# GeekAlexis/FastMOT

Hardware: AMD Instinct MI355X
Metric: end-to-end tracker FPS @1080p/50 dets (higher is better)
Workload: dtype f16

## Files before the change

### fastmot_amd/csrc/net.h

```cpp
#pragma once
#include "common.h"
#include <hip/hip_fp16.h>

typedef _Float16 f16;
typedef f16 f16x8 __attribute__((ext_vector_type(8)));
typedef f16 f16x4 __attribute__((ext_vector_type(4)));
typedef float f32x16 __attribute__((ext_vector_type(16)));
typedef float f32x4 __attribute__((ext_vector_type(4)));

enum { ACT_LINEAR = 0, ACT_LEAKY = 1, ACT_MISH = 2, ACT_RELU = 3, ACT_LOGISTIC = 4, ACT_SWISH = 5, ACT_RELU6 = 6 };
enum { RES_NONE = 0, RES_AFTER_ACT = 1, RES_BEFORE_ACT = 2 };

struct ConvParams {
    const f16* in;  int in_cs, in_coff;
    const f16* w;
    const float* bias;
    f16* out;       int out_cs, out_coff;
    float* out32;
    const f16* res; int res_cs, res_coff;
    int N, H, W, Cin, Ho, Wo, Cout, KH, KW, stride, pad;
    int K, Kpad, P;
    int cout_store;
    int act, res_mode;
    int grid_p, grid_c, grid_z, weight_major;
    int pad_dx;
    int up;
    int batch_inv;
};

int launch_conv(const ConvParams& p, float* ws, size_t ws_floats, hipStream_t s);

struct NetState {
    int which = 0, max_batch = 0;
    std::vector<fm_tensor> tensors;
    std::vector<void*> bufs;
    std::vector<fm_layer> layers;
    char* weights = nullptr;
    size_t weight_bytes = 0;
    float* gates = nullptr;
    int n_gates = 0, gate_c = 0;
    hipStream_t stream = nullptr;
    char* arena = nullptr;
    float* ws = nullptr;
    size_t ws_floats = 0;
    std::vector<std::pair<long, hipGraphExec_t>> graphs;
    bool use_graphs = true;
    int emb_offset = 0;
    int batch_offset = 0;
    int first = 0;
};

NetState* fm_net_get(fm_ctx* ctx, int which);
int fm_net_run_internal(fm_ctx* ctx, int which, int batch);

__device__ __forceinline__ void unpack8(const uint4& v, float* f) {
    const f16x8 h = *reinterpret_cast<const f16x8*>(&v);
#pragma unroll
    for (int e = 0; e < 8; ++e) f[e] = (float)h[e];
}
__device__ __forceinline__ uint4 pack8(const float* f) {
    f16x8 h;
#pragma unroll
    for (int e = 0; e < 8; ++e) h[e] = (f16)f[e];
    return *reinterpret_cast<const uint4*>(&h);
// ... 107 lines not shown
```

### fastmot_amd/csrc/net.hip

```cpp
#include "pixel_source.h"
#include <algorithm>
#include <memory>

int launch_dwconv3(const f16* in, int in_cs, int in_coff, f16* out, int out_cs, int out_coff, const f16* w,
                   const float* bias, int N, int H, int W, int C, int act, hipStream_t s);
int launch_dwconv(const f16* in, int in_cs, int in_coff, f16* out, int out_cs, int out_coff, const f16* w,
                  const float* bias, int N, int H, int W, int Ho, int Wo, int C, int stride, int act, hipStream_t s);
bool sepconv_supported(int cin, int cout, int stride);
int launch_sepconv(const f16* in, int in_cs, int in_coff, f16* out, int out_cs, int out_coff, const f16* wdw,
                   const float* bdw, const f16* wpw, const float* bpw, int N, int H, int W, int Ho, int Wo, int cin,
                   int cout, int stride, int act1, int act2, long p_choice, hipStream_t s);
int launch_liteconv(int G, const f16* const* in, const int* in_cs, const int* in_coff, f16* out, int out_cs,
                    int out_coff, const f16* wpw, int kpad, const f16* wdw, const float* bias, int N, int H,
                    int W, int C, int act, float* gap_out, hipStream_t s);
void liteconv_tiling(int C, int W, int H, int* th, int* tw, int* tiles_x, int* tiles_y);
int launch_litechain(const f16* in, int in_cs, int in_coff, f16* out, int out_cs, int out_coff, const f16* wpw,
                     int kpad, const f16* wdw, const float* bias, int N, int H, int W, int C, int act,
                     float* const* gap, hipStream_t s);
int launch_gated_sum(int nstreams, const f16* const* in, const int* in_cs, const int* in_coff, int N, int HW,
                     int C, int hid, const f16* w1, const float* b1, const f16* w2, const float* b2, f16* out,
                     int out_cs, int out_coff, const float* const* part, int tiles, hipStream_t s);
constexpr int GATE_SLOT_TILES = 32;
int launch_pair11(const f16* xa, int xa_cs, int xa_coff, const f16* xc, int xc_cs, int xc_coff, f16* out, int out_cs,
                  int out_coff, const f16* w1, const float* b1, const f16* w2, const float* b2, long P, int cout, int act1,
// ... 4 lines not shown
bool ostail_supported(int in_h, int in_w, int cin, int mid, int cout, int feat, int n_halfs, int n_floats);
int launch_stemconv(const f16* in, int in_cs, int in_coff, f16* out, int out_cs, int out_coff, const f16* w,
                    const float* bias, int N, int H, int W, int Ho, int Wo, int k, int stride, int pad, int cout,
                    int act, hipStream_t s);
int launch_spp(const f16* in, int in_cs, int in_coff, f16* out, int out_cs, int out_coff, int N, int H, int W,
               int C, hipStream_t s);
int launch_pool(const f16* in, int in_cs, int in_coff, f16* out, int out_cs, int out_coff, int N, int H,
                int W, int C, int Ho, int Wo, int k, int stride, int pad, int avg, hipStream_t s);
int launch_upsample2(const f16* in, int in_cs, int in_coff, f16* out, int out_cs, int out_coff, int N, int H,
                     int W, int C, hipStream_t s);
int launch_conv_streamed(const ConvParams& p, hipStream_t s);
int launch_convd(const ConvParams& p, hipStream_t s);
bool resblock_supported(int C, int M);
int launch_resblock(const f16* x, int x_cs, int x_coff, f16* out, int out_cs, int out_coff, const f16* w1,
                    const float* b1, const f16* w2, const float* b2, int N, int H, int W, int C, int M, int act1,
                    int act2, hipStream_t s);
int launch_add(const f16* a, int a_cs, int a_coff, const f16* b, int b_cs, int b_coff, f16* out, int out_cs,
               int out_coff, long npix, int C, hipStream_t s);
int launch_copy(const f16* in, int in_cs, int in_coff, f16* out, int out_cs, int out_coff, long npix, int C,
                hipStream_t s);
int launch_gate(const f16* in, int in_cs, int in_coff, int N, int HW, int C, int hid, const f16* w1,
                const float* b1, const f16* w2, const float* b2, float* gate, hipStream_t s);
int launch_gate_sum(int nstreams, const f16* const* in, const int* in_cs, const int* in_coff,
                    const float* const* gate, f16* out, int out_cs, int out_coff, int N, int HW, int C,
                    hipStream_t s);
int launch_head(const f16* in, int in_cs, int in_coff, int N, int HW, int C, int D, const f16* w,
                const float* b, float* out, float* raw_out, hipStream_t s, float* mirror = nullptr);
int launch_poolhead(const f16* in, int in_cs, int in_coff, int N, int HW, int C, int D, const float* scale, const float* shift,
                    const f16* w, const float* b, int relu, float* out, float* mirror, hipStream_t s);
int fm_emb_reserve(fm_ctx* ctx, int n);

// ... 23 lines not shown
    for (auto& g : net->graphs) (void)hipGraphExecDestroy(g.second);
    net->graphs.clear();
}

static size_t elem_size(const fm_tensor& t) { return t.f32 ? 4 : 2; }

extern "C" int fm_net_destroy(fm_ctx* ctx, int which) {
    FM_CHECK_ARG(ctx && (which >= 0 && which < FM_NET_EXTRACTOR_B + FM_MAX_EXTRA_EXTRACTORS));
    NetState*& slot = net_slot(ctx, which);
    if (slot) {
        FM_HIP(hipStreamSynchronize(slot->stream));
        fm_net_free(slot);
        slot = nullptr;
    }
    return 0;
}

extern "C" int fm_net_create(fm_ctx* ctx, int which, int max_batch, int n_tensors, const fm_tensor* tensors,
                             int n_layers, const fm_layer* layers, const void* weights, size_t weight_bytes,
                             int n_gates, int gate_channels, size_t arena_bytes) {
    FM_CHECK_ARG(ctx && (which >= 0 && which < FM_NET_EXTRACTOR_B + FM_MAX_EXTRA_EXTRACTORS) && max_batch > 0 && n_tensors > 0 && n_layers > 0);
    FM_CHECK_ARG(tensors && layers && weights && weight_bytes > 0);
    int rc = fm_net_destroy(ctx, which);
    if (rc) return rc;
    std::unique_ptr<NetState, void (*)(NetState*)> net(new NetState(), fm_net_free);
    net->which = which;
    net->max_batch = max_batch;
    net->stream = which == FM_NET_DETECTOR ? ctx->s_det : which == FM_NET_EXTRACTOR ? ctx->s_ext
                                                        : ctx->s_ext_x[which - FM_NET_EXTRACTOR_B];
    net->tensors.assign(tensors, tensors + n_tensors);
// ... 27 lines not shown
    FM_HIP(hipMalloc(&net->weights, weight_bytes));
    FM_HIP(hipMemcpy(net->weights, weights, weight_bytes, hipMemcpyHostToDevice));
    net->weight_bytes = weight_bytes;
    net->n_gates = n_gates;
    net->gate_c = gate_channels;
    net->ws_floats = ((size_t)16 << 20) * (which == FM_NET_DETECTOR ? (size_t)std::min(max_batch, FM_MAX_DET_BATCH) : 1);
    FM_HIP(hipMalloc(&net->ws, net->ws_floats * sizeof(float)));
    if (n_gates > 0) {
        FM_CHECK_ARG(gate_channels > 0);
        FM_HIP(hipMalloc(&net->gates, sizeof(float) * (size_t)n_gates * max_batch * gate_channels * GATE_SLOT_TILES));
    }
    if (which != FM_NET_DETECTOR) {
        FM_HIP(hipStreamSynchronize(ctx->s_main));
        if ((rc = fm_emb_reserve(ctx, max_batch))) return rc;
    }
    net_slot(ctx, which) = net.release();
    return 0;
}

static int run_layer(fm_ctx* ctx, NetState* net, const fm_layer& L, int B) {
    const fm_tensor& ti = net->tensors[L.in[0]];
    const fm_tensor& to = net->tensors[L.out];
    hipStream_t s = net->stream;
    float* ws = net->ws;
    const f16* in0 = (const f16*)net->bufs[L.in[0]];
    f16* out = (f16*)net->bufs[L.out];
    switch (L.op) {
        case FM_OP_CONV:
        case FM_OP_CONVS:
        case FM_OP_CONVD: {
            ConvParams p{};
            p.in = in0; p.in_cs = ti.c; p.in_coff = L.in_coff[0];
            p.w = (const f16*)(net->weights + L.w_off);
            p.bias = (const float*)(net->weights + L.b_off);
            p.out = to.f32 ? nullptr : out;
// ... 137 lines not shown
            FM_CHECK_ARG(to.h == ti.h && to.w == ti.w && L.out_coff + 3 * L.cin <= to.c);
            return launch_spp(in0, ti.c, L.in_coff[0], out, to.c, L.out_coff, B, ti.h, ti.w, L.cin, s);
        case FM_OP_MAXPOOL:
        case FM_OP_AVGPOOL:
            return launch_pool(in0, ti.c, L.in_coff[0], out, to.c, L.out_coff, B, ti.h, ti.w, L.cin, to.h, to.w,
                               L.k, L.stride, L.pad, L.op == FM_OP_AVGPOOL, s);
        case FM_OP_UPSAMPLE2:
            FM_CHECK_ARG(to.h == 2 * ti.h && to.w == 2 * ti.w);
            return launch_upsample2(in0, ti.c, L.in_coff[0], out, to.c, L.out_coff, B, ti.h, ti.w, L.cin, s);
        case FM_OP_RESBLOCK:
            FM_CHECK_ARG(!to.f32 && to.h == ti.h && to.w == ti.w && L.cin == L.cout &&
                         L.in_coff[0] + L.cin <= ti.c && L.out_coff + L.cout <= to.c);
            return launch_resblock(in0, ti.c, L.in_coff[0], out, to.c, L.out_coff,
                                   (const f16*)(net->weights + L.w_off), (const float*)(net->weights + L.b_off),
                                   (const f16*)(net->weights + L.w2_off), (const float*)(net->weights + L.b2_off),
                                   B, ti.h, ti.w, L.cin, L.hid, L.act, L.act, s);
        case FM_OP_ADD: {
            FM_CHECK_ARG(L.n_in == 2);
            const fm_tensor& tb = net->tensors[L.in[1]];
            FM_CHECK_ARG(tb.h == ti.h && tb.w == ti.w && to.h == ti.h && to.w == ti.w);
            return launch_add(in0, ti.c, L.in_coff[0], (const f16*)net->bufs[L.in[1]], tb.c, L.in_coff[1], out, to.c,
                              L.out_coff, (long)B * ti.h * ti.w, L.cin, s);
        }
        case FM_OP_COPY:
            return launch_copy(in0, ti.c, L.in_coff[0], out, to.c, L.out_coff, (long)B * ti.h * ti.w, L.cin, s);
        case FM_OP_GATE:
            FM_CHECK_ARG(L.gate[0] >= 0 && L.gate[0] < net->n_gates && L.cin <= net->gate_c);
            return launch_gate(in0, ti.c, L.in_coff[0], B, ti.h * ti.w, L.cin, L.hid,
                               (const f16*)(net->weights + L.w_off), (const float*)(net->weights + L.b_off),
                               (const f16*)(net->weights + L.w2_off), (const float*)(net->weights + L.b2_off),
                               net->gates + (size_t)L.gate[0] * net->max_batch * net->gate_c * GATE_SLOT_TILES, s);
// ... 39 lines not shown
                                   ctx->emb_host ? ctx->emb_host + (size_t)net->emb_offset * ctx->feat_dim : nullptr, s);
        }
        default:
            fm_set_error("unknown layer op %d", L.op);
            return FM_ERR_ARG;
    }
}

bool fm_net_writes_mirror(const NetState* net) {
    if (!net || net->layers.empty()) return false;
    const int op = net->layers.back().op;
    return op == FM_OP_HEAD || op == FM_OP_OSTAIL || op == FM_OP_POOLHEAD;
}

static int run_layers_eager(fm_ctx* ctx, NetState* net, int batch) {
    for (size_t i = (size_t)net->first; i < net->layers.size(); ++i) {
        int rc = run_layer(ctx, net, net->layers[i], batch);
        if (rc) return rc;
    }
    return 0;
}

bool fm_net_stem_fusable(const NetState* net, int input_tensor) {
    if (!net || net->layers.empty()) return false;
    const fm_layer& L = net->layers[0];
    if ((L.op != FM_OP_STEMCONV && L.op != FM_OP_STEM2 && L.op != FM_OP_STEMPOOL) || L.n_in != 1 || L.in[0] != input_tensor || L.in_coff[0] != 0) return false;
    for (size_t i = 1; i < net->layers.size(); ++i) {
        const fm_layer& M = net->layers[i];
        for (int k = 0; k < M.n_in; ++k)
            if (M.in[k] == input_tensor) return false;
        if (M.res_mode != FM_RES_NONE && M.res == input_tensor) return false;
        if (M.out == input_tensor) return false;
    }
// ... 295 lines not shown
```

### fastmot_amd/csrc/pair11.hip

```cpp
#include "net.h"

namespace {

template <int COUT, int PT>
__global__ __launch_bounds__(256) void pair11_kernel(const f16* __restrict__ xa, int xa_cs, int xa_coff,
                                                     const f16* __restrict__ xc, int xc_cs, int xc_coff,
                                                     f16* __restrict__ out, int out_cs, int out_coff,
                                                     const f16* __restrict__ w1, const float* __restrict__ b1,
                                                     const f16* __restrict__ w2, const float* __restrict__ b2,
                                                     long P, int act1, int act2) {
    constexpr int C = 64, S = C + 8, BN = 32 * PT, NCT = COUT / 32, WPT = 4 / PT, NM = 2 / WPT, NC = NCT / WPT;
    constexpr int NLD = BN * 8 / 256;
    __shared__ __attribute__((aligned(16))) f16 ta[BN * S];
    __shared__ __attribute__((aligned(16))) f16 tc[BN * S];
    const int tid = threadIdx.x, lane = tid & 63, wave = __builtin_amdgcn_readfirstlane(tid >> 6);
    const int frow = lane & 31, fh = lane >> 5;
    const int pt = wave % PT, part = wave / PT;
    const long p0 = (long)blockIdx.x * BN;

    f16x8 fa1[NM][4];
#pragma unroll
    for (int m = 0; m < NM; ++m)
#pragma unroll
        for (int q = 0; q < 4; ++q)
// ... 10 lines not shown
    for (int i = 0; i < NLD; ++i) {
        const int e = tid + i * 256, row = e >> 3, c8 = (e & 7) * 8;
        *reinterpret_cast<f16x8*>(&ta[row * S + c8]) = va[i];
        *reinterpret_cast<f16x8*>(&tc[row * S + c8]) = vc[i];
    }
    float4 bias1[NM][4];
#pragma unroll
    for (int m = 0; m < NM; ++m)
#pragma unroll
        for (int g = 0; g < 4; ++g) bias1[m][g] = *reinterpret_cast<const float4*>(b1 + (part * NM + m) * 32 + g * 8 + fh * 4);
    __syncthreads();

    const f16* brow = ta + (pt * 32 + frow) * S + fh * 8;
    f32x16 acc1[NM];
#pragma unroll
    for (int m = 0; m < NM; ++m)
#pragma unroll
        for (int r = 0; r < 16; ++r) acc1[m][r] = 0.f;
#pragma unroll
    for (int q = 0; q < 4; ++q) {
        const f16x8 fb = *reinterpret_cast<const f16x8*>(brow + q * 16);
#pragma unroll
        for (int m = 0; m < NM; ++m) acc1[m] = __builtin_amdgcn_mfma_f32_32x32x16_f16(fa1[m][q], fb, acc1[m], 0, 0, 0);
    }
    if constexpr (WPT > 1) __syncthreads(); else __builtin_amdgcn_wave_barrier();
#pragma unroll
    for (int m = 0; m < NM; ++m)
#pragma unroll
        for (int g = 0; g < 4; ++g) {
            const float4 bv = bias1[m][g];
            float a4[4] = {acc1[m][4 * g + 0] + bv.x, acc1[m][4 * g + 1] + bv.y, acc1[m][4 * g + 2] + bv.z,
                           acc1[m][4 * g + 3] + bv.w};
            apply_act_n<4>(a4, act1);
            union { f16 h[4]; uint2 u; } pk;
#pragma unroll
            for (int e = 0; e < 4; ++e) pk.h[e] = (f16)a4[e];
            *reinterpret_cast<uint2*>(&ta[(pt * 32 + frow) * S + (part * NM + m) * 32 + g * 8 + fh * 4]) = pk.u;
        }
    if constexpr (WPT > 1) __syncthreads(); else __builtin_amdgcn_wave_barrier();

    const f16* crow = tc + (pt * 32 + frow) * S + fh * 8;
    const long pix = p0 + pt * 32 + frow;
#pragma unroll
    for (int c = 0; c < NC; ++c) {
        const int ct = part * NC + c;
        f16x8 fa2[8];
#pragma unroll
        for (int q = 0; q < 8; ++q) fa2[q] = *reinterpret_cast<const f16x8*>(w2 + (((long)ct * 8 + q) * 64 + lane) * 8);
        float4 bias2[4];
#pragma unroll
        for (int g = 0; g < 4; ++g) bias2[g] = *reinterpret_cast<const float4*>(b2 + ct * 32 + g * 8 + fh * 4);
        f32x16 acc;
#pragma unroll
        for (int r = 0; r < 16; ++r) acc[r] = 0.f;
#pragma unroll
        for (int q = 0; q < 4; ++q)
            acc = __builtin_amdgcn_mfma_f32_32x32x16_f16(fa2[q], *reinterpret_cast<const f16x8*>(brow + q * 16), acc, 0, 0, 0);
#pragma unroll
        for (int q = 0; q < 4; ++q)
            acc = __builtin_amdgcn_mfma_f32_32x32x16_f16(fa2[4 + q], *reinterpret_cast<const f16x8*>(crow + q * 16), acc, 0, 0, 0);
        if (pix < P) {
            f16* dst = out + pix * out_cs + out_coff + ct * 32;
#pragma unroll
            for (int g = 0; g < 4; ++g) {
                float a4[4] = {acc[4 * g + 0] + bias2[g].x, acc[4 * g + 1] + bias2[g].y, acc[4 * g + 2] + bias2[g].z,
                               acc[4 * g + 3] + bias2[g].w};
                apply_act_n<4>(a4, act2);
                f16x4 o;
#pragma unroll
                for (int e = 0; e < 4; ++e) o[e] = (f16)a4[e];
                *reinterpret_cast<f16x4*>(dst + g * 8 + fh * 4) = o;
            }
        }
    }
}

template <int COUT, int PT>
int launch_pt(const f16* xa, int xa_cs, int xa_coff, const f16* xc, int xc_cs, int xc_coff, f16* out, int out_cs,
              int out_coff, const f16* w1, const float* b1, const f16* w2, const float* b2, long P, int act1, int act2,
              hipStream_t s) {
    const dim3 grid((unsigned)((P + 32 * PT - 1) / (32 * PT))), block(256);
    hipLaunchKernelGGL((pair11_kernel<COUT, PT>), grid, block, 0, s, xa, xa_cs, xa_coff, xc, xc_cs, xc_coff, out, out_cs, out_coff,
                       w1, b1, w2, b2, P, act1, act2);
    FM_HIP(hipGetLastError());
    return 0;
}

// ... 16 lines not shown
```

### fastmot_amd/csrc/resblock.hip

```cpp
#include "net.h"
#include <cstdlib>

namespace {

typedef float f32x16 __attribute__((ext_vector_type(16)));

template <int C, int M, int TH, int NW, int CS, int KS>
__global__ __launch_bounds__(NW * 64) void resblock_kernel(
    const f16* __restrict__ x, int x_cs, int x_coff, f16* __restrict__ out, int out_cs, int out_coff,
    const f16* __restrict__ w1, const float* __restrict__ b1, const f16* __restrict__ w2,
    const float* __restrict__ b2, int H, int W, int tiles_x, int act1, int act2) {
    constexpr int TW = 8, HW = TW + 2, NPOS = (TH + 2) * HW, SX = C + 8, S = M + 8, NT = NW * 64;
    constexpr int NMT = M / 32, NPH = (NPOS + 31) / 32, NPAIR = NMT * NPH / NW;
    constexpr int NCT = C / 32 / CS, NPT = TH * TW / 32;
    static_assert(NMT * NPH % NW == 0 && NCT * NPT * KS == NW, "tile / wave split");
    extern __shared__ __attribute__((aligned(16))) f16 lds[];
    f16* xt = lds;
    f16* mid = lds + NPOS * SX;
    const int tid = threadIdx.x, lane = tid & 63, wave = __builtin_amdgcn_readfirstlane(tid >> 6);
    const int frow = lane & 31, fk = (lane >> 5) * 8;
    const int tile = blockIdx.x / CS, cs = blockIdx.x % CS;
    const int ty0 = (tile / tiles_x) * TH, tx0 = (tile % tiles_x) * TW;
    const long n = blockIdx.y;
    const f16* img = x + n * (long)H * W * x_cs + x_coff;

    {
        constexpr int VPP = C / 8, NV = NPOS * VPP, NIT = (NV + NT - 1) / NT;
        f16x8 v[NIT];
#pragma unroll
        for (int i = 0; i < NIT; ++i) {
            const int e = tid + i * NT, pos = e / VPP, c8 = (e % VPP) * 8;
            const int py = ty0 - 1 + pos / HW, px = tx0 - 1 + pos % HW;
            const bool ok = e < NV && py >= 0 && py < H && px >= 0 && px < W;
            const f16x8 ld = *reinterpret_cast<const f16x8*>(
                img + ((long)min(max(py, 0), H - 1) * W + min(max(px, 0), W - 1)) * x_cs + c8);
#pragma unroll
            for (int j = 0; j < 8; ++j) v[i][j] = ok ? ld[j] : (f16)0.f;
        }
#pragma unroll
        for (int i = 0; i < NIT; ++i) {
            const int e = tid + i * NT;
            if (e < NV) *reinterpret_cast<f16x8*>(&xt[(e / VPP) * SX + (e % VPP) * 8]) = v[i];
        }
    }

    {
        constexpr int ST = C / 16, CH1 = ST < 8 ? ST : 8, KC = ST / CH1, NI = NPAIR * KC, PD = NI < 3 ? NI : 3;
        f16x8 fa[PD][CH1];
        float4 bias1[NPAIR][4];
#pragma unroll
        for (int p = 0; p < NPAIR; ++p)
#pragma unroll
            for (int g = 0; g < 4; ++g)
                bias1[p][g] = *reinterpret_cast<const float4*>((const float*)__builtin_assume_aligned(b1, 16) +
                                                               ((wave + p * NW) % NMT) * 32 + g * 8 + (lane >> 5) * 4);
        auto load_a = [&](int item, int slot) {
            const int mt = (wave + (item / KC) * NW) % NMT;
// ... 73 lines not shown
#pragma unroll
        for (int r = 0; r < 16; ++r) acc[r] = 0.f;
        __syncthreads();
        load_b(0, 0);
#pragma unroll
        for (int q = 0; q < NQ; ++q) {
            if (q + 1 < NQ) load_b(q + 1, (q + 1) & 1);
            __builtin_amdgcn_sched_barrier(0);
#pragma unroll
            for (int u = 0; u < CH; ++u)
                acc = __builtin_amdgcn_mfma_f32_32x32x16_f16(fa[q % PD][u], fb[q & 1][u], acc, 0, 0, 0);
            if (q + PD < NQ) load_a(q + PD, q % PD);
            __builtin_amdgcn_sched_barrier(0);
        }
    }
    if constexpr (KS > 1) {
        float4* red = reinterpret_cast<float4*>(mid);
        __syncthreads();
        if (ks > 0) {
#pragma unroll
            for (int g = 0; g < 4; ++g)
                red[(((ks - 1) * NCT * NPT + ctl + NCT * pt) * 4 + g) * 64 + lane] =
                    make_float4(acc[g * 4], acc[g * 4 + 1], acc[g * 4 + 2], acc[g * 4 + 3]);
        }
        __syncthreads();
        if (ks > 0) return;
#pragma unroll
        for (int k = 1; k < KS; ++k)
#pragma unroll
            for (int g = 0; g < 4; ++g) {
                const float4 v = red[(((k - 1) * NCT * NPT + ctl + NCT * pt) * 4 + g) * 64 + lane];
                acc[g * 4] += v.x; acc[g * 4 + 1] += v.y; acc[g * 4 + 2] += v.z; acc[g * 4 + 3] += v.w;
            }
    }

    if (gy < H && gx < W) {
        const long gp = (n * H + gy) * (long)W + gx;
        const f16* rsrc = xt + ((pix / TW + 1) * HW + pix % TW + 1) * SX;
#pragma unroll
        for (int g = 0; g < 4; ++g) {
            const int co = ct * 32 + g * 8 + (lane >> 5) * 4;
            const f16x4 rv = *reinterpret_cast<const f16x4*>(rsrc + co);
            f16x4 o;
            float a4[4] = {acc[g * 4 + 0] + bias2[g].x, acc[g * 4 + 1] + bias2[g].y, acc[g * 4 + 2] + bias2[g].z,
                           acc[g * 4 + 3] + bias2[g].w};
            apply_act_n<4>(a4, act2);
#pragma unroll
            for (int e = 0; e < 4; ++e) o[e] = (f16)(a4[e] + (float)rv[e]);
            *reinterpret_cast<f16x4*>(out + gp * out_cs + out_coff + co) = o;
        }
    }
}

template <int C, int M, int TH, int NW, int KS>
constexpr size_t resblock_lds() {
    constexpr size_t npos = (TH + 2) * 10, midb = npos * (M + 8) * 2, redb = (size_t)(KS - 1) * (NW / KS) * 64 * 64;
    return npos * (C + 8) * 2 + (midb > redb ? midb : redb);
}

template <int C, int M, int TH, int NW, int CS, int KS>
int resblock_launch(const f16* x, int x_cs, int x_coff, f16* out, int out_cs, int out_coff, const f16* w1,
                    const float* b1, const f16* w2, const float* b2, int N, int H, int W, int act1, int act2,
                    hipStream_t s) {
    const int tiles_x = (W + 7) / 8, tiles_y = (H + TH - 1) / TH;
    constexpr size_t shmem = resblock_lds<C, M, TH, NW, KS>();
    static_assert(shmem <= 64 * 1024, "LDS tile");
    hipLaunchKernelGGL((resblock_kernel<C, M, TH, NW, CS, KS>), dim3(tiles_x * tiles_y * CS, N), dim3(NW * 64), shmem, s, x, x_cs,
                       x_coff, out, out_cs, out_coff, w1, b1, w2, b2, H, W, tiles_x, act1, act2);
    FM_HIP(hipGetLastError());
    return 0;
}

}

bool resblock_supported(int C, int M) {
    return (C == 64 || C == 128 || C == 256) && (M == C || M == C / 2);
}

int launch_resblock(const f16* x, int x_cs, int x_coff, f16* out, int out_cs, int out_coff, const f16* w1,
                    const float* b1, const f16* w2, const float* b2, int N, int H, int W, int C, int M, int act1,
                    int act2, hipStream_t s) {
    FM_CHECK_ARG(resblock_supported(C, M) && x_cs % 8 == 0 && x_coff % 8 == 0 && out_cs % 4 == 0 && out_coff % 4 == 0);
#define RB(C_, M_, TH_, NW_, CS_, KS_)                                                                         \
    if (C == C_ && M == M_)                                                                                    \
        return resblock_launch<C_, M_, TH_, NW_, CS_, KS_>(x, x_cs, x_coff, out, out_cs, out_coff, w1, b1, w2, \
                                                           b2, N, H, W, act1, act2, s)
    static const int variant = getenv("FASTMOT_RB_VARIANT") ? atoi(getenv("FASTMOT_RB_VARIANT")) : 1;
    if (variant == 1) { RB(64, 64, 8, 8, 1, 2); RB(128, 128, 4, 8, 1, 2); }
    if (variant == 2) { RB(128, 128, 8, 8, 1, 1); }
    RB(64, 32, 8, 4, 1, 1);
    RB(64, 64, 8, 4, 1, 1);
    RB(128, 64, 4, 4, 1, 1);
    RB(128, 128, 4, 4, 1, 1);
    RB(256, 128, 4, 8, 4, 4);
    RB(256, 256, 4, 8, 4, 4);
#undef RB
    return FM_ERR_ARG;
}

extern "C" int fm_resblock_supported(int c, int mid) { return resblock_supported(c, mid) ? 1 : 0; }
```

### fastmot_amd/engine.py

```python
import ctypes as C

import numpy as np

from . import _lib

NET_DETECTOR, NET_EXTRACTOR, NET_EXTRACTOR_B = 0, 1, 2


class HipNet:
    def __init__(self, ctx, which, graph, max_batch, reuse_buffers=False):
        self.ctx, self.which, self.graph, self.max_batch = ctx, which, graph, max_batch
        ts, ls, blob = graph.tables(max_batch, reuse_buffers)
        self._keep = (ts, ls, blob)
        _lib.check(ctx.lib.fm_net_create(ctx.handle, C.c_int(which), C.c_int(max_batch), C.c_int(len(ts)), ts,
                                         C.c_int(len(ls)), ls, blob, C.c_size_t(len(blob)),
                                         C.c_int(graph.n_gates), C.c_int(graph.gate_c),
                                         C.c_size_t(graph.arena_bytes)))

    def run(self, batch):
        _lib.check(self.ctx.lib.fm_net_run(self.ctx.handle, C.c_int(self.which), C.c_int(batch)))

    def write(self, view, array):
        h, w, cpad, f32 = self.graph.tensors[view.tid]
        assert view.coff == 0 and not f32
# ... 13 lines not shown
    def read_embeddings(self, n):
        out = np.empty((n, self.ctx.feat_dim), np.float32)
        _lib.check(self.ctx.lib.fm_net_read_embeddings(self.ctx.handle, C.c_int(n), out.ctypes.data_as(C.c_void_p)))
        return out

    def read_embeddings_mirror(self, n):
        out = np.empty((n, self.ctx.feat_dim), np.float32)
        _lib.check(self.ctx.lib.fm_net_read_embeddings_mirror(self.ctx.handle, C.c_int(n), out.ctypes.data_as(C.c_void_p)))
        return out

    def cost(self, batch):
        f, b = C.c_double(0), C.c_double(0)
        _lib.check(self.ctx.lib.fm_net_cost(self.ctx.handle, C.c_int(self.which), C.c_int(batch), C.byref(f), C.byref(b)))
        return f.value, b.value

    def profile(self, batch, iters=3):
        conv_ms, other_ms = C.c_double(0), C.c_double(0)
        n_conv, n_other = C.c_int(0), C.c_int(0)
        _lib.check(self.ctx.lib.fm_net_profile(self.ctx.handle, C.c_int(self.which), C.c_int(batch), C.c_int(iters),
                                               C.byref(conv_ms), C.byref(other_ms), C.byref(n_conv), C.byref(n_other)))
        return dict(conv_ms=conv_ms.value, other_ms=other_ms.value, n_conv=n_conv.value, n_other=n_other.value)

    def profile_layers(self, batch, iters=5):
        out = np.zeros(len(self.graph.layers))
        _lib.check(self.ctx.lib.fm_net_profile_layers(self.ctx.handle, C.c_int(self.which), C.c_int(batch), C.c_int(iters),
                                                      out.ctypes.data_as(C.c_void_p)))
        return out

    def close(self):
        _lib.check(self.ctx.lib.fm_net_destroy(self.ctx.handle, C.c_int(self.which)))
# ... 1 lines not shown
```

### fastmot_amd/models/graph.py

```python
import ctypes as C
import logging
import os

import numpy as np

LOGGER = logging.getLogger(__name__)

(OP_CONV, OP_DWCONV3, OP_MAXPOOL, OP_AVGPOOL, OP_UPSAMPLE2, OP_COPY, OP_GATE, OP_GATE_SUM, OP_HEAD,
 OP_LITECONV, OP_SPP, OP_GATED_SUM, OP_STEMCONV, OP_ADD, OP_RESBLOCK, OP_CONVS, OP_LITECHAIN, OP_CONVD, OP_STEM2, OP_PAIR11,
 OP_OSTAIL, OP_DWCONV, OP_SEPCONV, OP_POOLHEAD, OP_STEMPOOL) = range(25)
CONV_OPS = (OP_CONV, OP_CONVS, OP_CONVD)
SPP_MAX_HW = 2048
ACT = {'linear': 0, 'leaky': 1, 'mish': 2, 'relu': 3, 'logistic': 4, 'swish': 5, 'relu6': 6}
RES_NONE, RES_AFTER_ACT, RES_BEFORE_ACT = 0, 1, 2


class fm_tensor(C.Structure):
    _fields_ = [('h', C.c_int32), ('w', C.c_int32), ('c', C.c_int32), ('f32', C.c_int32), ('offset', C.c_int64)]


class fm_layer(C.Structure):
    _fields_ = [('op', C.c_int32), ('n_in', C.c_int32),
                ('in_', C.c_int32 * 4), ('in_coff', C.c_int32 * 4),
                ('out', C.c_int32), ('out_coff', C.c_int32),
# ... 679 lines not shown
        else:
            assert not relu
        dst = View(x.tid, x.coff, x.c, x.h, x.w)
        self._layer(op=OP_POOLHEAD, ins=[x], out=dst, cin=c, cout=dim, act=ACT['relu' if relu else 'linear'],
                    gates=[int(neck is not None), int(fc is not None)], name=name, poolhead_ref=tuple(ref), **kw)
        return dst

    def plan_arena(self, max_batch, reuse):
        n = len(self.tensors)
        size = [ceil_to(max_batch * h * w * c * (4 if f32 else 2), 256) for (h, w, c, f32) in self.tensors]
        first, last = [10**9] * n, [-1] * n
        for li, d in enumerate(self.layers):
            touched = [v.tid for v in d['ins']] + [d['out'].tid] + ([d['res'].tid] if d['res'] is not None else [])
            for t in touched:
                first[t], last[t] = min(first[t], li), max(last[t], li)
        persistent = {self.input.tid} | {v.tid for v in self.outputs}
        for t in range(n):
            if t in persistent or not reuse or last[t] < 0:
                first[t], last[t] = -1, 10**9

        def disjoint(t, u):
            if first[t] < 0 or first[u] < 0:
                return False
            return last[t] < first[u] or last[u] < first[t]
        offsets = [0] * n
        placed = []
        for t in sorted(range(n), key=lambda i: -size[i]):
            cands = sorted((o, s) for (o, s, u) in placed if not disjoint(t, u))
            off = 0
            for o, s in cands:
# ... 63 lines not shown
```

### include/fastmot_hip.h

```cpp
#ifndef FASTMOT_HIP_H
#define FASTMOT_HIP_H

#include <stddef.h>
#include <stdint.h>

#ifdef __cplusplus
extern "C" {
#endif

typedef struct fm_ctx fm_ctx;

int fm_ctx_create(int device, fm_ctx** out);
int fm_ctx_destroy(fm_ctx* ctx);
const char* fm_last_error(void);
int fm_device_count(void);
int fm_device_pci_bus_id(int device, char* buf, int buflen);
int fm_ctx_synchronize(fm_ctx* ctx);
int fm_ctx_bind_thread(fm_ctx* ctx);
int fm_ctx_set_option(fm_ctx* ctx, const char* key, int value);
int fm_trace_start(fm_ctx* ctx, int cap, int64_t* host_ns);
int fm_trace_read(fm_ctx* ctx, int cap, int32_t* tags, float* ms, int* n);
int fm_device_info(fm_ctx* ctx, char* buf, int buflen);

typedef struct fm_kf_params {
// ... 142 lines not shown
    int64_t w_off, b_off, w2_off, b2_off;
} fm_layer;

int fm_net_create(fm_ctx* ctx, int which, int max_batch, int n_tensors, const fm_tensor* tensors,
                  int n_layers, const fm_layer* layers, const void* weights, size_t weight_bytes,
                  int n_gates, int gate_channels, size_t arena_bytes);
int fm_net_destroy(fm_ctx* ctx, int which);
int fm_net_run(fm_ctx* ctx, int which, int batch);
int fm_net_tensor_write(fm_ctx* ctx, int which, int tensor, const void* host, size_t bytes);
int fm_net_tensor_read(fm_ctx* ctx, int which, int tensor, void* host, size_t bytes);
int fm_net_read_embeddings(fm_ctx* ctx, int n, float* host);
int fm_net_read_embeddings_mirror(fm_ctx* ctx, int n, float* host);
int fm_net_cost(fm_ctx* ctx, int which, int batch, double* flops, double* bytes);
int fm_net_profile(fm_ctx* ctx, int which, int batch, int iters, double* conv_ms, double* other_ms,
                   int* n_conv, int* n_other);

int fm_net_profile_layers(fm_ctx* ctx, int which, int batch, int iters, double* out);

int fm_frame_configure(fm_ctx* ctx, int width, int height, int ring_size);
int fm_frame_upload(fm_ctx* ctx, const uint8_t* bgr);
int fm_host_alloc(size_t bytes, void** out);
int fm_host_free(void* p);
int fm_frame_upload_next(fm_ctx* ctx, const uint8_t* bgr);
int fm_frame_ring_select_next(fm_ctx* ctx, int index);
int fm_frame_promote_next(fm_ctx* ctx);
int fm_detect_async_next(fm_ctx* ctx);
#define FM_MAX_DET_BATCH 4
int fm_frame_upload_ahead(fm_ctx* ctx, int k, const uint8_t* bgr);
int fm_frame_ring_select_ahead(fm_ctx* ctx, int k, int index);
int fm_detect_async_ahead(fm_ctx* ctx, int n);
// ... 324 lines not shown
```

Measured before the change: 1015.

## Fuse following pointwise convolutions into the resblock kernel tail

New measurement: 1031, median of 6. 1.6% higher.

```diff
diff --git a/fastmot_amd/csrc/net.h b/fastmot_amd/csrc/net.h
--- a/fastmot_amd/csrc/net.h
+++ b/fastmot_amd/csrc/net.h
@@ -30,6 +30,22 @@
 
 int launch_conv(const ConvParams& p, float* ws, size_t ws_floats, hipStream_t s);
 
+struct ResblockTail {
+    const f16* xc;  int xc_cs, xc_coff;
+    f16* t;         int t_cs, t_coff;
+    f16* out;       int out_cs, out_coff;
+    const f16* w1;  const float* b1;
+    const f16* w2;  const float* b2;
+    int act1, act2, cout;
+    int wfmt;
+};
+
+struct LaunchPlan {
+    std::vector<unsigned char> span;
+    std::vector<ResblockTail> tail;
+    int launches = 0;
+};
+
 struct NetState {
     int which = 0, max_batch = 0;
     std::vector<fm_tensor> tensors;
@@ -48,6 +64,7 @@
     int emb_offset = 0;
     int batch_offset = 0;
     int first = 0;
+    LaunchPlan plan;
 };
 
 NetState* fm_net_get(fm_ctx* ctx, int which);
diff --git a/fastmot_amd/csrc/net.hip b/fastmot_amd/csrc/net.hip
--- a/fastmot_amd/csrc/net.hip
+++ b/fastmot_amd/csrc/net.hip
@@ -1,5 +1,7 @@
 #include "pixel_source.h"
+#include "pointwise_mfma.h"
 #include <algorithm>
+#include <cstdlib>
 #include <memory>
 
 int launch_dwconv3(const f16* in, int in_cs, int in_coff, f16* out, int out_cs, int out_coff, const f16* w,
@@ -42,7 +44,8 @@
 bool resblock_supported(int C, int M);
 int launch_resblock(const f16* x, int x_cs, int x_coff, f16* out, int out_cs, int out_coff, const f16* w1,
                     const float* b1, const f16* w2, const float* b2, int N, int H, int W, int C, int M, int act1,
-                    int act2, hipStream_t s);
+                    int act2, hipStream_t s, const ResblockTail* tail = nullptr);
+bool resblock_tail_supported(int C, int M, int cout, int wfmt);
 int launch_add(const f16* a, int a_cs, int a_coff, const f16* b, int b_cs, int b_coff, f16* out, int out_cs,
                int out_coff, long npix, int C, hipStream_t s);
 int launch_copy(const f16* in, int in_cs, int in_coff, f16* out, int out_cs, int out_coff, long npix, int C,
@@ -96,6 +99,93 @@
         slot = nullptr;
     }
     return 0;
+}
+
+static int launch_fuse_mask() {
+    const char* e = getenv("FASTMOT_LAUNCH_FUSE");
+    return e && *e ? (int)strtol(e, nullptr, 0) : 7;
+}
+
+static bool views_overlap(const NetState* net, int ta, int ca, int na, int tb, int cb, int nb) {
+    if (ta == tb) return ca < cb + nb && cb < ca + na;
+    auto bytes = [&](int t) {
+        const fm_tensor& T = net->tensors[t];
+        return (size_t)net->max_batch * T.h * T.w * T.c * elem_size(T);
+    };
+    const char* a = (const char*)net->bufs[ta];
+    const char* b = (const char*)net->bufs[tb];
+    return a < b + bytes(tb) && b < a + bytes(ta);
+}
+
+static int plan_tail(const NetState* net, size_t i, int mask, ResblockTail* tail) {
+    const fm_layer& L = net->layers[i];
+    if (L.op != FM_OP_RESBLOCK || i + 1 >= net->layers.size() || L.cin != L.cout) return 0;
+    const int bit = L.cin == 64 ? (L.hid == 32 ? 1 : L.hid == 64 ? 2 : 0) : (L.cin == 128 && L.hid == 128 ? 4 : 0);
+    if (!(mask & bit)) return 0;
+    const fm_tensor& ty = net->tensors[L.out];
+    const int C = L.cin;
+    auto same_map = [&](int t) { const fm_tensor& T = net->tensors[t]; return T.h == ty.h && T.w == ty.w && !T.f32; };
+    auto blob = [&](int64_t off) { return net->weights + off; };
+    ResblockTail tl{};
+    int n = 0, t_tensor = -1, xc_tensor, out_tensor;
+    const fm_layer& P = net->layers[i + 1];
+    if (P.op == FM_OP_PAIR11) {
+        if (!(P.n_in == 2 && P.in[0] == L.out && P.in_coff[0] == L.out_coff && P.cin == C && P.hid == C &&
+              pair11_supported(P.cin, P.hid, P.cin, P.cout) && resblock_tail_supported(C, L.hid, P.cout, PW_W_FRAG) &&
+              same_map(P.in[1]) && same_map(P.out) && P.in_coff[1] + C <= net->tensors[P.in[1]].c &&
+              P.out_coff + P.cout <= net->tensors[P.out].c))
+            return 0;
+        n = 1;
+        xc_tensor = P.in[1]; out_tensor = P.out;
+        tl.xc = (const f16*)net->bufs[P.in[1]]; tl.xc_cs = net->tensors[P.in[1]].c; tl.xc_coff = P.in_coff[1];
+        tl.out = (f16*)net->bufs[P.out]; tl.out_cs = net->tensors[P.out].c; tl.out_coff = P.out_coff;
+        tl.w1 = (const f16*)blob(P.w_off); tl.b1 = (const float*)blob(P.b_off);
+        tl.w2 = (const f16*)blob(P.w2_off); tl.b2 = (const float*)blob(P.b2_off);
+        tl.act1 = P.gate[0]; tl.act2 = P.act; tl.cout = P.cout; tl.wfmt = PW_W_FRAG;
+    } else {
+        if (i + 2 >= net->layers.size()) return 0;
+        const fm_layer& Q = net->layers[i + 2];
+        auto pointwise = [&](const fm_layer& K, int cin, int cout) {
+            return K.op == FM_OP_CONVD && K.n_in == 1 && K.k == 1 && K.stride == 1 && K.pad == 0 && K.res_mode == FM_RES_NONE &&
+                   K.up <= 1 && K.cin == cin && K.cout == cout && same_map(K.in[0]) && same_map(K.out) &&
+                   K.in_coff[0] + cin <= net->tensors[K.in[0]].c && K.out_coff + cout <= net->tensors[K.out].c;
+        };
+        if (!(pointwise(P, C, C) && pointwise(Q, 2 * C, 2 * C) && P.in[0] == L.out && P.in_coff[0] == L.out_coff &&
+              Q.in[0] == P.out && Q.in_coff[0] == P.out_coff && resblock_tail_supported(C, L.hid, Q.cout, PW_W_TILE64)))
+            return 0;
+        n = 2;
+        t_tensor = xc_tensor = P.out; out_tensor = Q.out;
+        tl.t = (f16*)net->bufs[P.out]; tl.t_cs = net->tensors[P.out].c; tl.t_coff = P.out_coff;
+        tl.xc = tl.t; tl.xc_cs = tl.t_cs; tl.xc_coff = P.out_coff + C;
+        tl.out = (f16*)net->bufs[Q.out]; tl.out_cs = net->tensors[Q.out].c; tl.out_coff = Q.out_coff;
+        tl.w1 = (const f16*)blob(P.w_off); tl.b1 = (const float*)blob(P.b_off);
+        tl.w2 = (const f16*)blob(Q.w_off); tl.b2 = (const float*)blob(Q.b_off);
+        tl.act1 = P.act; tl.act2 = Q.act; tl.cout = Q.cout; tl.wfmt = PW_W_TILE64;
+    }
+    struct V { int t, c, n; };
+    const V x{L.in[0], L.in_coff[0], C}, y{L.out, L.out_coff, C}, xc{xc_tensor, tl.xc_coff, C}, out{out_tensor, tl.out_coff, tl.cout};
+    const V t{t_tensor, tl.t_coff, C};
+    auto hit = [&](const V& a, const V& b) { return views_overlap(net, a.t, a.c, a.n, b.t, b.c, b.n); };
+    if (hit(y, x) || hit(y, xc) || hit(out, x) || hit(out, xc) || hit(out, y)) return 0;
+    if (t_tensor >= 0 && (hit(t, x) || hit(t, xc) || hit(t, y) || hit(t, out))) return 0;
+    *tail = tl;
+    return n;
+}
+
+static void plan_launches(NetState* net) {
+    const size_t n = net->layers.size();
+    LaunchPlan& plan = net->plan;
+    plan.span.assign(n, 1);
+    plan.tail.assign(n, ResblockTail{});
+    plan.launches = 0;
+    const int mask = launch_fuse_mask();
+    for (size_t i = 0; i < n;) {
+        const int absorbed = mask ? plan_tail(net, i, mask, &plan.tail[i]) : 0;
+        plan.span[i] = (unsigned char)(1 + absorbed);
+        for (int k = 1; k <= absorbed; ++k) plan.span[i + k] = 0;
+        ++plan.launches;
+        i += 1 + absorbed;
+    }
 }
 
 extern "C" int fm_net_create(fm_ctx* ctx, int which, int max_batch, int n_tensors, const fm_tensor* tensors,
@@ -153,11 +243,20 @@
         FM_HIP(hipStreamSynchronize(ctx->s_main));
         if ((rc = fm_emb_reserve(ctx, max_batch))) return rc;
     }
+    plan_launches(net.get());
     net_slot(ctx, which) = net.release();
     return 0;
 }
 
-static int run_layer(fm_ctx* ctx, NetState* net, const fm_layer& L, int B) {
+extern "C" int fm_net_launch_count(fm_ctx* ctx, int which, int* launches) {
+    FM_CHECK_ARG(ctx && (which >= 0 && which < FM_NET_EXTRACTOR_B + FM_MAX_EXTRA_EXTRACTORS) && launches);
+    NetState* net = net_slot(ctx, which);
+    FM_CHECK_ARG(net != nullptr);
+    *launches = net->plan.launches;
+    return 0;
+}
+
+static int run_layer(fm_ctx* ctx, NetState* net, const fm_layer& L, int B, const ResblockTail* tail = nullptr) {
     const fm_tensor& ti = net->tensors[L.in[0]];
     const fm_tensor& to = net->tensors[L.out];
     hipStream_t s = net->stream;
@@ -325,7 +424,7 @@
             return launch_resblock(in0, ti.c, L.in_coff[0], out, to.c, L.out_coff,
                                    (const f16*)(net->weights + L.w_off), (const float*)(net->weights + L.b_off),
                                    (const f16*)(net->weights + L.w2_off), (const float*)(net->weights + L.b2_off),
-                                   B, ti.h, ti.w, L.cin, L.hid, L.act, L.act, s);
+                                   B, ti.h, ti.w, L.cin, L.hid, L.act, L.act, s, tail);
         case FM_OP_ADD: {
             FM_CHECK_ARG(L.n_in == 2);
             const fm_tensor& tb = net->tensors[L.in[1]];
@@ -395,9 +494,12 @@
 }
 
 static int run_layers_eager(fm_ctx* ctx, NetState* net, int batch) {
-    for (size_t i = (size_t)net->first; i < net->layers.size(); ++i) {
-        int rc = run_layer(ctx, net, net->layers[i], batch);
+    const LaunchPlan& plan = net->plan;
+    for (size_t i = (size_t)net->first; i < net->layers.size();) {
+        const int span = std::max<int>(plan.span[i], 1);
+        int rc = run_layer(ctx, net, net->layers[i], batch, span > 1 ? &plan.tail[i] : nullptr);
         if (rc) return rc;
+        i += span;
     }
     return 0;
 }
diff --git a/fastmot_amd/csrc/pair11.hip b/fastmot_amd/csrc/pair11.hip
--- a/fastmot_amd/csrc/pair11.hip
+++ b/fastmot_amd/csrc/pair11.hip
@@ -1,4 +1,4 @@
-#include "net.h"
+#include "pointwise_mfma.h"
 
 namespace {
 
@@ -48,29 +48,18 @@
     const f16* brow = ta + (pt * 32 + frow) * S + fh * 8;
     f32x16 acc1[NM];
 #pragma unroll
-    for (int m = 0; m < NM; ++m)
+    for (int m = 0; m < NM; ++m) {
 #pragma unroll
         for (int r = 0; r < 16; ++r) acc1[m][r] = 0.f;
-#pragma unroll
-    for (int q = 0; q < 4; ++q) {
-        const f16x8 fb = *reinterpret_cast<const f16x8*>(brow + q * 16);
-#pragma unroll
-        for (int m = 0; m < NM; ++m) acc1[m] = __builtin_amdgcn_mfma_f32_32x32x16_f16(fa1[m][q], fb, acc1[m], 0, 0, 0);
+        acc1[m] = pw_mfma_run<4>(fa1[m], brow, acc1[m]);
     }
     if constexpr (WPT > 1) __syncthreads(); else __builtin_amdgcn_wave_barrier();
 #pragma unroll
     for (int m = 0; m < NM; ++m)
 #pragma unroll
-        for (int g = 0; g < 4; ++g) {
-            const float4 bv = bias1[m][g];
-            float a4[4] = {acc1[m][4 * g + 0] + bv.x, acc1[m][4 * g + 1] + bv.y, acc1[m][4 * g + 2] + bv.z,
-                           acc1[m][4 * g + 3] + bv.w};
-            apply_act_n<4>(a4, act1);
-            union { f16 h[4]; uint2 u; } pk;
-#pragma unroll
-            for (int e = 0; e < 4; ++e) pk.h[e] = (f16)a4[e];
-            *reinterpret_cast<uint2*>(&ta[(pt * 32 + frow) * S + (part * NM + m) * 32 + g * 8 + fh * 4]) = pk.u;
-        }
+        for (int g = 0; g < 4; ++g)
+            *reinterpret_cast<f16x4*>(&ta[(pt * 32 + frow) * S + (part * NM + m) * 32 + g * 8 + fh * 4]) =
+                pw_finish4(acc1[m], g, bias1[m][g], act1);
     if constexpr (WPT > 1) __syncthreads(); else __builtin_amdgcn_wave_barrier();
 
     const f16* crow = tc + (pt * 32 + frow) * S + fh * 8;
@@ -87,24 +76,12 @@
         f32x16 acc;
 #pragma unroll
         for (int r = 0; r < 16; ++r) acc[r] = 0.f;
-#pragma unroll
-        for (int q = 0; q < 4; ++q)
-            acc = __builtin_amdgcn_mfma_f32_32x32x16_f16(fa2[q], *reinterpret_cast<const f16x8*>(brow + q * 16), acc, 0, 0, 0);
-#pragma unroll
-        for (int q = 0; q < 4; ++q)
-            acc = __builtin_amdgcn_mfma_f32_32x32x16_f16(fa2[4 + q], *reinterpret_cast<const f16x8*>(crow + q * 16), acc, 0, 0, 0);
+        acc = pw_mfma_run<4>(fa2, brow, acc);
+        acc = pw_mfma_run<4>(fa2 + 4, crow, acc);
         if (pix < P) {
             f16* dst = out + pix * out_cs + out_coff + ct * 32;
 #pragma unroll
-            for (int g = 0; g < 4; ++g) {
-                float a4[4] = {acc[4 * g + 0] + bias2[g].x, acc[4 * g + 1] + bias2[g].y, acc[4 * g + 2] + bias2[g].z,
-                               acc[4 * g + 3] + bias2[g].w};
-                apply_act_n<4>(a4, act2);
-                f16x4 o;
-#pragma unroll
-                for (int e = 0; e < 4; ++e) o[e] = (f16)a4[e];
-                *reinterpret_cast<f16x4*>(dst + g * 8 + fh * 4) = o;
-            }
+            for (int g = 0; g < 4; ++g) *reinterpret_cast<f16x4*>(dst + g * 8 + fh * 4) = pw_finish4(acc, g, bias2[g], act2);
         }
     }
 }
diff --git a/fastmot_amd/csrc/pointwise_mfma.h b/fastmot_amd/csrc/pointwise_mfma.h
--- /dev/null
+++ b/fastmot_amd/csrc/pointwise_mfma.h
@@ -0,0 +1,35 @@
+#pragma once
+#include "net.h"
+
+enum {
+    PW_W_FRAG = 1,
+    PW_W_TILE64 = 2
+};
+
+template <int FMT>
+__device__ __forceinline__ f16x8 pw_wfrag(const f16* __restrict__ w, int ct, int nq, int q, int lane) {
+    if constexpr (FMT == PW_W_FRAG) {
+        return *reinterpret_cast<const f16x8*>(w + (((long)ct * nq + q) * 64 + lane) * 8);
+    } else {
+        const int row = lane & 31, chunk = 2 * (q & 3) + (lane >> 5);
+        return *reinterpret_cast<const f16x8*>(w + (((long)ct * (nq >> 2) + (q >> 2)) * 32 + row) * 64 +
+                                               ((chunk ^ ((row >> 1) & 7)) << 3));
+    }
+}
+
+template <int NQ>
+__device__ __forceinline__ f32x16 pw_mfma_run(const f16x8* fa, const f16* brow, f32x16 acc) {
+#pragma unroll
+    for (int q = 0; q < NQ; ++q)
+        acc = __builtin_amdgcn_mfma_f32_32x32x16_f16(fa[q], *reinterpret_cast<const f16x8*>(brow + q * 16), acc, 0, 0, 0);
+    return acc;
+}
+
+__device__ __forceinline__ f16x4 pw_finish4(const f32x16& acc, int g, const float4 bv, int act) {
+    float a4[4] = {acc[4 * g + 0] + bv.x, acc[4 * g + 1] + bv.y, acc[4 * g + 2] + bv.z, acc[4 * g + 3] + bv.w};
+    apply_act_n<4>(a4, act);
+    f16x4 o;
+#pragma unroll
+    for (int e = 0; e < 4; ++e) o[e] = (f16)a4[e];
+    return o;
+}
diff --git a/fastmot_amd/csrc/resblock.hip b/fastmot_amd/csrc/resblock.hip
--- a/fastmot_amd/csrc/resblock.hip
+++ b/fastmot_amd/csrc/resblock.hip
@@ -1,15 +1,23 @@
-#include "net.h"
+#include "pointwise_mfma.h"
 #include <cstdlib>
+#include <type_traits>
 
 namespace {
 
-typedef float f32x16 __attribute__((ext_vector_type(16)));
-
-template <int C, int M, int TH, int NW, int CS, int KS>
+struct RbNoTail {};
+
+template <int C, int M, int TH, int NW, int KS>
+constexpr size_t resblock_lds() {
+    constexpr size_t npos = (TH + 2) * 10, midb = npos * (M + 8) * 2, redb = (size_t)(KS - 1) * (NW / KS) * 64 * 64;
+    return npos * (C + 8) * 2 + (midb > redb ? midb : redb);
+}
+
+template <int C, int M, int TH, int NW, int CS, int KS, int TAIL = 0, int TC = 0>
 __global__ __launch_bounds__(NW * 64) void resblock_kernel(
     const f16* __restrict__ x, int x_cs, int x_coff, f16* __restrict__ out, int out_cs, int out_coff,
     const f16* __restrict__ w1, const float* __restrict__ b1, const f16* __restrict__ w2,
-    const float* __restrict__ b2, int H, int W, int tiles_x, int act1, int act2) {
+    const float* __restrict__ b2, int H, int W, int tiles_x, int act1, int act2,
+    const std::conditional_t<TAIL != 0, ResblockTail, RbNoTail> tl) {
     constexpr int TW = 8, HW = TW + 2, NPOS = (TH + 2) * HW, SX = C + 8, S = M + 8, NT = NW * 64;
     constexpr int NMT = M / 32, NPH = (NPOS + 31) / 32, NPAIR = NMT * NPH / NW;
     constexpr int NCT = C / 32 / CS, NPT = TH * TW / 32;
@@ -24,6 +32,20 @@
     const long n = blockIdx.y;
     const f16* img = x + n * (long)H * W * x_cs + x_coff;
 
+    constexpr int NPIX = TH * TW, XVPP = C / 8, XNV = NPIX * XVPP, XNIT = TAIL ? (XNV + NT - 1) / NT : 1;
+    static_assert(!TAIL || (CS == 1 && (C / 32) * (NPIX / 32) <= NW && (TC / 32) * (NPIX / 32) == NW), "tail tiles / waves");
+    f16* const xct = lds + resblock_lds<C, M, TH, NW, KS>() / 2;
+    f16x8 vx[XNIT];
+    if constexpr (TAIL != 0) {
+        const f16* ximg = tl.xc + n * (long)H * W * tl.xc_cs + tl.xc_coff;
+#pragma unroll
+        for (int i = 0; i < XNIT; ++i) {
+            const int e = min(tid + i * NT, XNV - 1), pix = e / XVPP;
+            vx[i] = *reinterpret_cast<const f16x8*>(
+                ximg + ((long)min(ty0 + pix / TW, H - 1) * W + min(tx0 + pix % TW, W - 1)) * tl.xc_cs + (e % XVPP) * 8);
+        }
+    }
+
     {
         constexpr int VPP = C / 8, NV = NPOS * VPP, NIT = (NV + NT - 1) / NT;
         f16x8 v[NIT];
@@ -41,6 +63,13 @@
         for (int i = 0; i < NIT; ++i) {
             const int e = tid + i * NT;
             if (e < NV) *reinterpret_cast<f16x8*>(&xt[(e / VPP) * SX + (e % VPP) * 8]) = v[i];
+        }
+    }
+    if constexpr (TAIL != 0) {
+#pragma unroll
+        for (int i = 0; i < XNIT; ++i) {
+            const int e = tid + i * NT;
+            if (e < XNV) *reinterpret_cast<f16x8*>(&xct[(e / XVPP) * SX + (e % XVPP) * 8]) = vx[i];
         }
     }
 
@@ -144,6 +173,20 @@
             __builtin_amdgcn_sched_barrier(0);
         }
     }
+    constexpr int NQ1 = C / 16, NMT1 = C / 32, NT1 = NMT1 * (NPIX / 32);
+    const int mt1 = wave % NMT1, pt1 = wave / NMT1;
+    f16x8 fa1[TAIL ? NQ1 : 1];
+    float4 tb1[4];
+    if constexpr (TAIL != 0) {
+        if (wave < NT1) {
+#pragma unroll
+            for (int q = 0; q < NQ1; ++q) fa1[q] = pw_wfrag<TAIL>(tl.w1, mt1, NQ1, q, lane);
+#pragma unroll
+            for (int g = 0; g < 4; ++g)
+                tb1[g] = *reinterpret_cast<const float4*>((const float*)__builtin_assume_aligned(tl.b1, 16) + mt1 * 32 + g * 8 +
+                                                          (lane >> 5) * 4);
+        }
+    }
     if constexpr (KS > 1) {
         float4* red = reinterpret_cast<float4*>(mid);
         __syncthreads();
@@ -154,19 +197,22 @@
                     make_float4(acc[g * 4], acc[g * 4 + 1], acc[g * 4 + 2], acc[g * 4 + 3]);
         }
         __syncthreads();
-        if (ks > 0) return;
-#pragma unroll
-        for (int k = 1; k < KS; ++k)
-#pragma unroll
-            for (int g = 0; g < 4; ++g) {
-                const float4 v = red[(((k - 1) * NCT * NPT + ctl + NCT * pt) * 4 + g) * 64 + lane];
-                acc[g * 4] += v.x; acc[g * 4 + 1] += v.y; acc[g * 4 + 2] += v.z; acc[g * 4 + 3] += v.w;
-            }
-    }
-
-    if (gy < H && gx < W) {
+        if (ks > 0) {
+            if constexpr (TAIL == 0) return;
+        } else {
+#pragma unroll
+            for (int k = 1; k < KS; ++k)
+#pragma unroll
+                for (int g = 0; g < 4; ++g) {
+                    const float4 v = red[(((k - 1) * NCT * NPT + ctl + NCT * pt) * 4 + g) * 64 + lane];
+                    acc[g * 4] += v.x; acc[g * 4 + 1] += v.y; acc[g * 4 + 2] += v.z; acc[g * 4 + 3] += v.w;
+                }
+        }
+    }
+
+    if ((TAIL == 0 || KS == 1 || ks == 0) && gy < H && gx < W) {
         const long gp = (n * H + gy) * (long)W + gx;
-        const f16* rsrc = xt + ((pix / TW + 1) * HW + pix % TW + 1) * SX;
+        f16* rsrc = xt + ((pix / TW + 1) * HW + pix % TW + 1) * SX;
 #pragma unroll
         for (int g = 0; g < 4; ++g) {
             const int co = ct * 32 + g * 8 + (lane >> 5) * 4;
@@ -178,25 +224,69 @@
 #pragma unroll
             for (int e = 0; e < 4; ++e) o[e] = (f16)(a4[e] + (float)rv[e]);
             *reinterpret_cast<f16x4*>(out + gp * out_cs + out_coff + co) = o;
-        }
-    }
-}
-
-template <int C, int M, int TH, int NW, int KS>
-constexpr size_t resblock_lds() {
-    constexpr size_t npos = (TH + 2) * 10, midb = npos * (M + 8) * 2, redb = (size_t)(KS - 1) * (NW / KS) * 64 * 64;
-    return npos * (C + 8) * 2 + (midb > redb ? midb : redb);
-}
-
-template <int C, int M, int TH, int NW, int CS, int KS>
+            if constexpr (TAIL != 0) *reinterpret_cast<f16x4*>(rsrc + co) = o;
+        }
+    }
+
+    if constexpr (TAIL != 0) {
+        constexpr int NQ2 = 2 * NQ1, NCT2 = TC / 32;
+        const int fh = lane >> 5;
+        const int ct2 = wave % NCT2, pt2 = wave / NCT2;
+        f16x8 fa2[NQ2];
+#pragma unroll
+        for (int q = 0; q < NQ2; ++q) fa2[q] = pw_wfrag<TAIL>(tl.w2, ct2, NQ2, q, lane);
+        float4 tb2[4];
+#pragma unroll
+        for (int g = 0; g < 4; ++g)
+            tb2[g] = *reinterpret_cast<const float4*>((const float*)__builtin_assume_aligned(tl.b2, 16) + ct2 * 32 + g * 8 + fh * 4);
+        __syncthreads();
+        const int p1 = pt1 * 32 + frow;
+        f16* yrow = xt + ((p1 / TW + 1) * HW + p1 % TW + 1) * SX;
+        f32x16 acc1;
+#pragma unroll
+        for (int r = 0; r < 16; ++r) acc1[r] = 0.f;
+        if (wave < NT1) acc1 = pw_mfma_run<NQ1>(fa1, yrow + fk, acc1);
+        __syncthreads();
+        if (wave < NT1) {
+            const int py = ty0 + p1 / TW, px = tx0 + p1 % TW;
+            const bool st = tl.t != nullptr && py < H && px < W;
+            f16* tdst = tl.t + ((n * H + py) * (long)W + px) * tl.t_cs + tl.t_coff + mt1 * 32;
+#pragma unroll
+            for (int g = 0; g < 4; ++g) {
+                const f16x4 o = pw_finish4(acc1, g, tb1[g], tl.act1);
+                *reinterpret_cast<f16x4*>(yrow + mt1 * 32 + g * 8 + fh * 4) = o;
+                if (st) *reinterpret_cast<f16x4*>(tdst + g * 8 + fh * 4) = o;
+            }
+        }
+        __syncthreads();
+        const int p2 = pt2 * 32 + frow;
+        const f16* trow = xt + ((p2 / TW + 1) * HW + p2 % TW + 1) * SX + fk;
+        const f16* crow = xct + p2 * SX + fk;
+        f32x16 acc2;
+#pragma unroll
+        for (int r = 0; r < 16; ++r) acc2[r] = 0.f;
+        acc2 = pw_mfma_run<NQ1>(fa2, trow, acc2);
+        acc2 = pw_mfma_run<NQ1>(fa2 + NQ1, crow, acc2);
+        const int oy = ty0 + p2 / TW, ox = tx0 + p2 % TW;
+        if (oy < H && ox < W) {
+            f16* dst = tl.out + ((n * H + oy) * (long)W + ox) * tl.out_cs + tl.out_coff + ct2 * 32;
+#pragma unroll
+            for (int g = 0; g < 4; ++g) *reinterpret_cast<f16x4*>(dst + g * 8 + fh * 4) = pw_finish4(acc2, g, tb2[g], tl.act2);
+        }
+    }
+}
+
+template <int C, int M, int TH, int NW, int CS, int KS, int TAIL = 0, int TC = 0>
 int resblock_launch(const f16* x, int x_cs, int x_coff, f16* out, int out_cs, int out_coff, const f16* w1,
                     const float* b1, const f16* w2, const float* b2, int N, int H, int W, int act1, int act2,
-                    hipStream_t s) {
+                    hipStream_t s, const ResblockTail* tail = nullptr) {
     const int tiles_x = (W + 7) / 8, tiles_y = (H + TH - 1) / TH;
-    constexpr size_t shmem = resblock_lds<C, M, TH, NW, KS>();
+    constexpr size_t shmem = resblock_lds<C, M, TH, NW, KS>() + (TAIL ? (size_t)TH * 8 * (C + 8) * 2 : 0);
     static_assert(shmem <= 64 * 1024, "LDS tile");
-    hipLaunchKernelGGL((resblock_kernel<C, M, TH, NW, CS, KS>), dim3(tiles_x * tiles_y * CS, N), dim3(NW * 64), shmem, s, x, x_cs,
-                       x_coff, out, out_cs, out_coff, w1, b1, w2, b2, H, W, tiles_x, act1, act2);
+    std::conditional_t<TAIL != 0, ResblockTail, RbNoTail> tl{};
+    if constexpr (TAIL != 0) tl = *tail;
+    hipLaunchKernelGGL((resblock_kernel<C, M, TH, NW, CS, KS, TAIL, TC>), dim3(tiles_x * tiles_y * CS, N), dim3(NW * 64), shmem, s, x,
+                       x_cs, x_coff, out, out_cs, out_coff, w1, b1, w2, b2, H, W, tiles_x, act1, act2, tl);
     FM_HIP(hipGetLastError());
     return 0;
 }
@@ -207,15 +297,41 @@
     return (C == 64 || C == 128 || C == 256) && (M == C || M == C / 2);
 }
 
+static int rb_variant() {
+    static const int variant = getenv("FASTMOT_RB_VARIANT") ? atoi(getenv("FASTMOT_RB_VARIANT")) : 1;
+    return variant;
+}
+
+bool resblock_tail_supported(int C, int M, int cout, int wfmt) {
+    if (C == 64 && M == 32) return cout == 64 && wfmt == PW_W_FRAG;
+    if (C == 64 && M == 64) return cout == 128 && wfmt == PW_W_FRAG && rb_variant() == 1;
+    if (C == 128 && M == 128) return cout == 256 && wfmt == PW_W_TILE64 && rb_variant() == 1;
+    return false;
+}
+
 int launch_resblock(const f16* x, int x_cs, int x_coff, f16* out, int out_cs, int out_coff, const f16* w1,
                     const float* b1, const f16* w2, const float* b2, int N, int H, int W, int C, int M, int act1,
-                    int act2, hipStream_t s) {
+                    int act2, hipStream_t s, const ResblockTail* tail) {
     FM_CHECK_ARG(resblock_supported(C, M) && x_cs % 8 == 0 && x_coff % 8 == 0 && out_cs % 4 == 0 && out_coff % 4 == 0);
+    if (tail) {
+        FM_CHECK_ARG(resblock_tail_supported(C, M, tail->cout, tail->wfmt) && tail->xc && tail->out && tail->w1 && tail->b1 &&
+                     tail->w2 && tail->b2 && tail->xc_cs % 8 == 0 && tail->xc_coff % 8 == 0 && tail->out_cs % 4 == 0 &&
+                     tail->out_coff % 4 == 0 && (!tail->t || (tail->t_cs % 4 == 0 && tail->t_coff % 4 == 0)));
+#define RBT(C_, M_, TH_, NW_, KS_, FMT_, TC_)                                                                               \
+    if (C == C_ && M == M_)                                                                                                \
+        return resblock_launch<C_, M_, TH_, NW_, 1, KS_, FMT_, TC_>(x, x_cs, x_coff, out, out_cs, out_coff, w1, b1, w2, b2, \
+                                                                    N, H, W, act1, act2, s, tail)
+        RBT(64, 32, 8, 4, 1, PW_W_FRAG, 64);
+        RBT(64, 64, 8, 8, 2, PW_W_FRAG, 128);
+        RBT(128, 128, 4, 8, 2, PW_W_TILE64, 256);
+#undef RBT
+        return FM_ERR_ARG;
+    }
 #define RB(C_, M_, TH_, NW_, CS_, KS_)                                                                         \
     if (C == C_ && M == M_)                                                                                    \
         return resblock_launch<C_, M_, TH_, NW_, CS_, KS_>(x, x_cs, x_coff, out, out_cs, out_coff, w1, b1, w2, \
                                                            b2, N, H, W, act1, act2, s)
-    static const int variant = getenv("FASTMOT_RB_VARIANT") ? atoi(getenv("FASTMOT_RB_VARIANT")) : 1;
+    const int variant = rb_variant();
     if (variant == 1) { RB(64, 64, 8, 8, 1, 2); RB(128, 128, 4, 8, 1, 2); }
     if (variant == 2) { RB(128, 128, 8, 8, 1, 1); }
     RB(64, 32, 8, 4, 1, 1);
diff --git a/fastmot_amd/engine.py b/fastmot_amd/engine.py
--- a/fastmot_amd/engine.py
+++ b/fastmot_amd/engine.py
@@ -51,6 +51,11 @@
         _lib.check(self.ctx.lib.fm_net_cost(self.ctx.handle, C.c_int(self.which), C.c_int(batch), C.byref(f), C.byref(b)))
         return f.value, b.value
 
+    def launch_count(self):
+        n = C.c_int(0)
+        _lib.check(self.ctx.lib.fm_net_launch_count(self.ctx.handle, C.c_int(self.which), C.byref(n)))
+        return n.value
+
     def profile(self, batch, iters=3):
         conv_ms, other_ms = C.c_double(0), C.c_double(0)
         n_conv, n_other = C.c_int(0), C.c_int(0)
diff --git a/fastmot_amd/models/graph.py b/fastmot_amd/models/graph.py
--- a/fastmot_amd/models/graph.py
+++ b/fastmot_amd/models/graph.py
@@ -717,6 +717,20 @@
             touched = [v.tid for v in d['ins']] + [d['out'].tid] + ([d['res'].tid] if d['res'] is not None else [])
             for t in touched:
                 first[t], last[t] = min(first[t], li), max(last[t], li)
+        for li, d in enumerate(self.layers):
+            if d['op'] != OP_RESBLOCK:
+                continue
+            nxt = self.layers[li + 1:li + 3]
+            y = d['out']
+            if nxt and nxt[0]['op'] == OP_PAIR11 and (nxt[0]['ins'][0].tid, nxt[0]['ins'][0].coff) == (y.tid, y.coff):
+                end = li + 1
+            elif len(nxt) == 2 and all(e['op'] == OP_CONVD and e['k'] == 1 and e['stride'] == 1 for e in nxt) and \
+                    (nxt[0]['ins'][0].tid, nxt[0]['ins'][0].coff) == (y.tid, y.coff) and nxt[1]['ins'][0].tid == nxt[0]['out'].tid:
+                end = li + 2
+            else:
+                continue
+            for t in (d['ins'][0].tid, y.tid):
+                last[t] = max(last[t], end)
         persistent = {self.input.tid} | {v.tid for v in self.outputs}
         for t in range(n):
             if t in persistent or not reuse or last[t] < 0:
diff --git a/include/fastmot_hip.h b/include/fastmot_hip.h
--- a/include/fastmot_hip.h
+++ b/include/fastmot_hip.h
@@ -180,6 +180,8 @@
 int fm_net_cost(fm_ctx* ctx, int which, int batch, double* flops, double* bytes);
 int fm_net_profile(fm_ctx* ctx, int which, int batch, int iters, double* conv_ms, double* other_ms,
                    int* n_conv, int* n_other);
+
+int fm_net_launch_count(fm_ctx* ctx, int which, int* launches);
 
 int fm_net_profile_layers(fm_ctx* ctx, int which, int batch, int iters, double* out);
 
```
